# akashsengupta1997/STRAPS-3DHumanShapePose

Measured on AMD Instinct MI355X. Metric: bodies/sec, higher is better.
Workload: dtype fp32 (encoder convolutions as exact bf16x3 operand splits (six bf16 products per term); in-step SMPL blend contraction and skinning as 3-product fp16 splits (fp16x3_lbs: 22-bit operands); fp32 accumulate throughout)

## Files before the change

straps-3dhumanshapepose_amd/csrc/elementwise.hip:

```cpp
#include "common.h"

namespace {

__global__ __launch_bounds__(256) void pack_krsc_kernel(const float* __restrict__ src, float* __restrict__ dst, int O, int C, int R, int S) {
    const long long i = (long long)blockIdx.x * 256 + threadIdx.x;
    const long long n = (long long)O * C * R * S;
    if (i >= n) return;
    const int c = (int)(i % C);
    long long t = i / C;
    const int s = (int)(t % S); t /= S;
    const int r = (int)(t % R);
    const int o = (int)(t / R);
    dst[i] = src[(((long long)o * C + c) * R + r) * S + s];
}

__global__ __launch_bounds__(256) void pack_crsk_flip_kernel(const float* __restrict__ src, float* __restrict__ dst, int O, int C, int R, int S) {
    const long long i = (long long)blockIdx.x * 256 + threadIdx.x;
    const long long n = (long long)O * C * R * S;
    if (i >= n) return;
    const int o = (int)(i % O);
    long long t = i / O;
    const int s = (int)(t % S); t /= S;
    const int r = (int)(t % R);
    const int c = (int)(t / R);
// ... 102 lines not shown
            for (int idx = tid; idx < nc * nr * (PK_T / 4); idx += 256) {
                const int o = (idx & (PK_T / 4 - 1)) * 4;
                const int k = idx >> 3;
                const int c = nr == PK_RS ? k / PK_RS : k / nr, j = k - c * nr;
                if (o < no) {
                    const float* t = tile + o * PK_LD + c * PK_RS + j;
                    const f32x4 v = {t[0], t[PK_LD], t[2 * PK_LD], t[3 * PK_LD]};
                    store_planes4(c3, ps, D.first + wk_index(c0 + c, RS - 1 - (rs0 + j), o0 + o, D.c, D.o), v);
                }
            }
        }
        __syncthreads();
    }
}

__global__ void bn_fold_kernel(const float* __restrict__ g, const float* __restrict__ b, const float* __restrict__ mean,
                               const float* __restrict__ var, float eps, float* __restrict__ scale, float* __restrict__ shift, int C) {
    const int c = blockIdx.x * blockDim.x + threadIdx.x;
    if (c >= C) return;
    const float sc = g[c] / sqrtf(var[c] + eps);
    scale[c] = sc;
    shift[c] = fmaf(-mean[c], sc, b[c]);
}

__global__ __launch_bounds__(256) void maxpool_kernel(const float* __restrict__ x, float* __restrict__ y, int B, int H, int W, int C,
                                                      int Ho, int Wo) {
    const int C4 = C >> 2;
    const long long n = (long long)B * Ho * Wo * C4;
    for (long long i = (long long)blockIdx.x * 256 + threadIdx.x; i < n; i += (long long)gridDim.x * 256) {
        const int c4 = (int)(i % C4);
        long long t = i / C4;
        const int wo = (int)(t % Wo); t /= Wo;
        const int ho = (int)(t % Ho);
        const int b = (int)(t / Ho);
        f32x4 m = {-INFINITY, -INFINITY, -INFINITY, -INFINITY};
#pragma unroll
        for (int r = 0; r < 3; ++r) {
            const int hi = 2 * ho - 1 + r;
            if ((unsigned)hi >= (unsigned)H) continue;
#pragma unroll
            for (int s = 0; s < 3; ++s) {
                const int wi = 2 * wo - 1 + s;
                if ((unsigned)wi >= (unsigned)W) continue;
                const f32x4 v = *reinterpret_cast<const f32x4*>(x + (((long long)b * H + hi) * W + wi) * C + c4 * 4);
#pragma unroll
                for (int e = 0; e < 4; ++e)
                    if (v[e] > m[e] || v[e] != v[e]) m[e] = v[e];
            }
        }
        *reinterpret_cast<f32x4*>(y + i * 4) = m;
    }
}

__global__ __launch_bounds__(256) void gap_kernel(const float* __restrict__ x, float* __restrict__ y, int B, int HW, int C) {
    const long long i = (long long)blockIdx.x * 256 + threadIdx.x;
    if (i >= (long long)B * C) return;
    const int c = (int)(i % C);
    const long long b = i / C;
    const float* p = x + b * HW * C + c;
    float s = 0.f;
    for (int k = 0; k < HW; ++k) s += p[(long long)k * C];
    y[i] = s / (float)HW;
}

__global__ __launch_bounds__(256) void bn_stats_finalize_kernel(const float* __restrict__ part, int nblocks, int C, double count,
                                                               const float* __restrict__ gamma, const float* __restrict__ beta, float eps,
                                                               float momentum, float* __restrict__ rmean, float* __restrict__ rvar,
                                                               float* __restrict__ scale, float* __restrict__ shift,
                                                               float* __restrict__ smean, float* __restrict__ sinv) {
    int c;
    double s1, s2;
    if (bn_partials_sum4(part, nblocks, C, s1, s2, c)) {
        const double mean = s1 / count;
        double var = s2 / count - mean * mean;
        if (var < 0.0) var = 0.0;
        const float inv = (float)(1.0 / sqrt(var + (double)eps));
        const float sc = gamma[c] * inv;
        scale[c] = sc;
        shift[c] = fmaf(-(float)mean, sc, beta[c]);
        if (smean) smean[c] = (float)mean;
        if (sinv) sinv[c] = inv;
        if (rmean) {
            const double unbiased = count > 1.0 ? var * count / (count - 1.0) : var;
            rmean[c] = fmaf(momentum, (float)mean, (1.f - momentum) * rmean[c]);
            rvar[c] = fmaf(momentum, (float)unbiased, (1.f - momentum) * rvar[c]);
        }
    }
}

__global__ __launch_bounds__(256) void bn_apply_kernel(const float* __restrict__ x, const float* __restrict__ scale,
                                                       const float* __restrict__ shift, const float* __restrict__ res, int relu,
                                                       float* __restrict__ y, u16* __restrict__ planes, long long ps, long long n4, int C4,
                                                       unsigned* __restrict__ bits, int tiled) {
    const long long first = (long long)blockIdx.x * 256 + threadIdx.x, step = (long long)gridDim.x * 256;
    const long long rows = n4 / C4;
    auto body = [&](long long i, long long r, int c4, const f32x4& sc, const f32x4& sh) {
        f32x4 v = *reinterpret_cast<const f32x4*>(x + i * 4);
#pragma unroll
        for (int q = 0; q < 4; ++q) v[q] = fmaf(v[q], sc[q], sh[q]);
        if (res) v += *reinterpret_cast<const f32x4*>(res + i * 4);
        if (relu) { v[0] = fmaxf(v[0], 0.f); v[1] = fmaxf(v[1], 0.f); v[2] = fmaxf(v[2], 0.f); v[3] = fmaxf(v[3], 0.f); }
        if (y) *reinterpret_cast<f32x4*>(y + i * 4) = v;
        if (planes) store_planes4_cm(planes, ps, r, c4 * 4, rows, v);
        if (bits) {
            unsigned wd = ((v[0] > 0.f ? 1u : 0u) | (v[1] > 0.f ? 2u : 0u) | (v[2] > 0.f ? 4u : 0u) | (v[3] > 0.f ? 8u : 0u)) << ((c4 & 7) * 4);
            wd |= __shfl_xor(wd, 1, 64);
            wd |= __shfl_xor(wd, 2, 64);
            wd |= __shfl_xor(wd, 4, 64);
            if ((c4 & 7) == 0) bits[r * (C4 >> 3) + (c4 >> 3)] = wd;
        }
    };
    if (tiled) {
        const int l = threadIdx.x & 63, w = threadIdx.x >> 6, wcg = tiled, ncb = (C4 >> 4) / wcg, trows = 16 / wcg;
        const int c4 = ((int)(blockIdx.x % ncb) * wcg + w % wcg) * 16 + (l >> 5) * 8 + (l & 7);
// ... 54 lines not shown

extern "C" int straps_pack_conv_weights_batched(const straps_pack_desc_t* descs, int n, long long total, void* stream) {
    STRAPS_REQUIRE(descs && n > 0 && total > 0, "straps_pack_conv_weights_batched: bad arguments");
    long long blocks = (total + PK_T * PK_T * PK_RS - 1) / (PK_T * PK_T * PK_RS);
    if (blocks > 8192) blocks = 8192;
    hipLaunchKernelGGL(pack_batched_kernel, dim3((unsigned)blocks), dim3(256), 0, (hipStream_t)stream, descs, n, (u16*)nullptr, (u16*)nullptr, 0LL);
    STRAPS_CHECK_LAUNCH("pack_batched_kernel");
    return STRAPS_OK;
}

extern "C" int straps_pack_conv_weights_batched_x3(const straps_pack_desc_t* descs, int n, long long total, unsigned short* krsc_planes,
                                                   unsigned short* crsk_planes, long long plane_stride, void* stream) {
    STRAPS_REQUIRE(descs && n > 0 && total > 0, "straps_pack_conv_weights_batched_x3: bad arguments");
    STRAPS_REQUIRE(krsc_planes || crsk_planes, "straps_pack_conv_weights_batched_x3: no planes given (use straps_pack_conv_weights_batched)");
    STRAPS_REQUIRE(plane_stride >= total && plane_stride % 8 == 0, "straps_pack_conv_weights_batched_x3: plane_stride must be >= total and a multiple of 8");
    STRAPS_REQUIRE((reinterpret_cast<uintptr_t>(krsc_planes) & 15) == 0 && (reinterpret_cast<uintptr_t>(crsk_planes) & 15) == 0,
                   "straps_pack_conv_weights_batched_x3: plane buffers must be 16-byte aligned");
    long long blocks = (total + PK_T * PK_T * PK_RS - 1) / (PK_T * PK_T * PK_RS);
    if (blocks > 8192) blocks = 8192;
    hipLaunchKernelGGL(pack_batched_kernel, dim3((unsigned)blocks), dim3(256), 0, (hipStream_t)stream, descs, n, krsc_planes, crsk_planes, plane_stride);
    STRAPS_CHECK_LAUNCH("pack_batched_kernel");
    return STRAPS_OK;
}

extern "C" int straps_bn_fold(const float* gamma, const float* beta, const float* mean, const float* var, float eps, float* scale,
                              float* shift, int c, void* stream) {
    STRAPS_REQUIRE(gamma && beta && mean && var && scale && shift && c > 0, "straps_bn_fold: bad arguments");
    hipLaunchKernelGGL(bn_fold_kernel, dim3((c + 255) / 256), dim3(256), 0, (hipStream_t)stream, gamma, beta, mean, var, eps, scale, shift, c);
    STRAPS_CHECK_LAUNCH("bn_fold_kernel");
    return STRAPS_OK;
}

extern "C" int straps_bn_fold_stats(const float* gamma, const float* beta, const float* mean, const float* var, float eps, float* scale,
                                    float* shift, float* save_mean, float* save_invstd, int c, void* stream) {
    STRAPS_REQUIRE(gamma && beta && mean && var && scale && shift && save_mean && save_invstd && c > 0, "straps_bn_fold_stats: bad arguments");
    hipLaunchKernelGGL(bn_fold_stats_kernel, dim3((c + 255) / 256), dim3(256), 0, (hipStream_t)stream, gamma, beta, mean, var, eps, scale, shift, save_mean,
                       save_invstd, c);
    STRAPS_CHECK_LAUNCH("bn_fold_stats_kernel");
    return STRAPS_OK;
}

extern "C" int straps_maxpool_fwd(const float* x, float* y, int batch, int h, int w, int c, void* stream) {
    STRAPS_REQUIRE(x && y && batch > 0 && h > 0 && w > 0 && c > 0 && (c & 3) == 0, "straps_maxpool_fwd: bad arguments (c%%4 must be 0)");
    const int Ho = (h + 2 - 3) / 2 + 1, Wo = (w + 2 - 3) / 2 + 1;
    const long long n = (long long)batch * Ho * Wo * (c >> 2);
    hipLaunchKernelGGL(maxpool_kernel, dim3(capped_grid(n)), dim3(256), 0, (hipStream_t)stream, x, y, batch, h, w, c, Ho, Wo);
    STRAPS_CHECK_LAUNCH("maxpool_kernel");
    return STRAPS_OK;
}

extern "C" int straps_gap_fwd(const float* x, float* y, int batch, int hw, int c, void* stream) {
    STRAPS_REQUIRE(x && y && batch > 0 && hw > 0 && c > 0, "straps_gap_fwd: bad arguments");
    const long long n = (long long)batch * c;
    hipLaunchKernelGGL(gap_kernel, dim3((unsigned)((n + 255) / 256)), dim3(256), 0, (hipStream_t)stream, x, y, batch, hw, c);
    STRAPS_CHECK_LAUNCH("gap_kernel");
    return STRAPS_OK;
}

extern "C" int straps_bn_stats_finalize(const float* stats_partial, int nblocks, int c, long long count, const float* gamma,
                                        const float* beta, float eps, float momentum, float* running_mean, float* running_var,
                                        float* scale, float* shift, float* save_mean, float* save_invstd, void* stream) {
    STRAPS_REQUIRE(stats_partial && gamma && beta && scale && shift && nblocks > 0 && c > 0 && count > 0, "straps_bn_stats_finalize: bad arguments");
    STRAPS_REQUIRE((running_mean == nullptr) == (running_var == nullptr), "straps_bn_stats_finalize: running stats must be given together");
    hipLaunchKernelGGL(bn_stats_finalize_kernel, dim3((c + 3) / 4), dim3(256), 0, (hipStream_t)stream, stats_partial, nblocks, c, (double)count, gamma, beta,
                       eps, momentum, running_mean, running_var, scale, shift, save_mean, save_invstd);
    STRAPS_CHECK_LAUNCH("bn_stats_finalize_kernel");
    return STRAPS_OK;
}

extern "C" int straps_bn_apply(const float* x, const float* scale, const float* shift, const float* residual, int relu, float* y,
                               long long rows, int c, void* stream) {
    STRAPS_REQUIRE(x && scale && shift && y && rows > 0 && c > 0 && (c & 3) == 0, "straps_bn_apply: bad arguments (c%%4 must be 0)");
    const long long n4 = rows * (c >> 2);
    hipLaunchKernelGGL(bn_apply_kernel, dim3(capped_grid(n4)), dim3(256), 0, (hipStream_t)stream, x, scale, shift, residual, relu, y, (u16*)nullptr, 0LL, n4, c >> 2, (unsigned*)nullptr, 0);
    STRAPS_CHECK_LAUNCH("bn_apply_kernel");
    return STRAPS_OK;
}

static int bn_apply_x3_impl(const char* who, const float* x, const float* scale, const float* shift, const float* residual, int relu, float* y,
                            unsigned short* y_planes, long long plane_stride, unsigned* relu_bits, long long rows, int c, void* stream) {
    STRAPS_REQUIRE(x && scale && shift && (y_planes || y) && rows > 0 && c > 0 && (c & 31) == 0, "%s: bad arguments (c%%32 must be 0: chunk-major planes; c=%d)", who, c);
    STRAPS_REQUIRE(!y_planes || (plane_stride >= rows * c && plane_stride % 8 == 0), "%s: plane_stride must be >= rows*c and a multiple of 8", who);
    const long long n4 = rows * (c >> 2);
    const int tiled = straps_bn_tiled(rows, c >> 2);
    hipLaunchKernelGGL(bn_apply_kernel, dim3(tiled ? straps_bn_tiled_grid(rows, c >> 2, tiled) : straps_grid256_rows(n4, c >> 2)), dim3(256), 0, (hipStream_t)stream, x, scale, shift,
                       residual, relu, y, y_planes, plane_stride, n4, c >> 2, relu_bits, tiled);
    STRAPS_CHECK_LAUNCH("bn_apply_kernel");
    return STRAPS_OK;
}

extern "C" int straps_bn_apply_x3(const float* x, const float* scale, const float* shift, const float* residual, int relu, float* y,
                                  unsigned short* y_planes, long long plane_stride, long long rows, int c, void* stream) {
    return bn_apply_x3_impl("straps_bn_apply_x3", x, scale, shift, residual, relu, y, y_planes, plane_stride, nullptr, rows, c, stream);
}

extern "C" int straps_bn_apply_bits_x3(const float* x, const float* scale, const float* shift, const float* residual, float* y,
                                       unsigned short* y_planes, long long plane_stride, unsigned* relu_bits, long long rows, int c, void* stream) {
    STRAPS_REQUIRE(relu_bits, "straps_bn_apply_bits_x3: null bit buffer");
    return bn_apply_x3_impl("straps_bn_apply_bits_x3", x, scale, shift, residual, 1, y, y_planes, plane_stride, relu_bits, rows, c, stream);
}
```

straps-3dhumanshapepose_amd/csrc/ief.hip:

```cpp
#include "common.h"

namespace {

constexpr int LW = 8;
__global__ __launch_bounds__(64 * LW) void linear_kernel(const float* __restrict__ x, int ldx, const float* __restrict__ w, int ldw,
                                                     const float* __restrict__ bias, const float* addend, float* out, int ldo,
                                                     int M, int N, int K, int relu) {
    __shared__ float red[LW][32][33];
    const int tid = threadIdx.x, lane = tid & 63, wave = tid >> 6;
    const int m0 = blockIdx.y * 32, n0 = blockIdx.x * 32;
    const int i = lane & 31, h = lane >> 5;
    const int mr = min(m0 + i, M - 1);
    const float* xp = x + (long long)mr * ldx + 4 * h;
    const float* wp = w + (long long)(n0 + i) * ldw + 4 * h;
    f32x16 acc;
#pragma unroll
    for (int r = 0; r < 16; ++r) acc[r] = 0.f;
    const int G = K >> 3;
#pragma unroll 4
    for (int g = wave; g < G; g += LW) {
        const f32x4 a = *reinterpret_cast<const f32x4*>(xp + 8 * g);
        const f32x4 b = *reinterpret_cast<const f32x4*>(wp + 8 * g);
#pragma unroll
        for (int e = 0; e < 4; ++e) acc = mfma32(a[e], b[e], acc);
    }
#pragma unroll
    for (int r = 0; r < 16; ++r) red[wave][mfma_row(r, lane)][i] = acc[r];
    __syncthreads();
#pragma unroll
    for (int q = 0; q < 1024 / (64 * LW); ++q) {
        const int idx = tid + 64 * LW * q;
        const int row = idx >> 5, col = idx & 31;
        const int m = m0 + row, n = n0 + col;
        if (m < M && n < N) {
            float v = ((red[0][row][col] + red[1][row][col]) + (red[2][row][col] + red[3][row][col])) +
                      ((red[4][row][col] + red[5][row][col]) + (red[6][row][col] + red[7][row][col]));
            if (bias) v += bias[n];
            if (addend) v += addend[(long long)m * ldo + n];
            if (relu) v = fmaxf(v, 0.f);
            out[(long long)m * ldo + n] = v;
        }
    }
}

__global__ __launch_bounds__(256) void broadcast_rows_kernel(const float* __restrict__ row, int cols, float* __restrict__ dst,
                                                             int ld_dst, int m) {
    const long long i = (long long)blockIdx.x * 256 + threadIdx.x;
    if (i >= (long long)m * ld_dst) return;
    const int c = (int)(i % ld_dst);
    dst[i] = c < cols ? row[c] : 0.f;
}

struct GemmBatch {
    straps_gemm_desc_t d[STRAPS_GEMM_MULTI_MAX];
};

__global__ __launch_bounds__(64 * LW) void gemm_multi_kernel(GemmBatch batch) {
    const straps_gemm_desc_t& p = batch.d[blockIdx.z];
    const int M = p.m, N = p.n, K = p.k;
    const int m0 = blockIdx.y * 32, n0 = blockIdx.x * 32;
    if (m0 >= M || n0 >= N) return;
    __shared__ float red[LW][32][33];
    const int lane = threadIdx.x & 63, wave = threadIdx.x >> 6;
    const int i = lane & 31, h = lane >> 5;
    const int mr = min(m0 + i, M - 1), nr = min(n0 + i, N - 1);
    const float* ap = p.a + (long long)mr * p.sam;
    const float* bp = p.b + (long long)nr * p.sbn;
    const long long sak = p.sak, sbk = p.sbk;
    f32x16 acc;
#pragma unroll
    for (int q = 0; q < 16; ++q) acc[q] = 0.f;
    const int G = (K + 7) >> 3;
    for (int g = wave; g < G; g += 2 * LW) {
        float av[8], bv[8];
#pragma unroll
        for (int u = 0; u < 2; ++u) {
#pragma unroll
            for (int e = 0; e < 4; ++e) {
                const int k = (g + LW * u) * 8 + 4 * h + e;
                const bool ok = k < K;
                av[u * 4 + e] = ok ? ap[(long long)k * sak] : 0.f;
                bv[u * 4 + e] = ok ? bp[(long long)k * sbk] : 0.f;
            }
        }
#pragma unroll
        for (int e = 0; e < 8; ++e) acc = mfma32(av[e], bv[e], acc);
    }
#pragma unroll
    for (int q = 0; q < 16; ++q) red[wave][mfma_row(q, lane)][i] = acc[q];
    __syncthreads();
#pragma unroll
    for (int q = 0; q < 1024 / (64 * LW); ++q) {
        const int idx = threadIdx.x + 64 * LW * q;
        const int row = idx >> 5, col = idx & 31;
        const int m = m0 + row, n = n0 + col;
        if (m < M && n < N) {
            float v = ((red[0][row][col] + red[1][row][col]) + (red[2][row][col] + red[3][row][col])) +
                      ((red[4][row][col] + red[5][row][col]) + (red[6][row][col] + red[7][row][col]));
            if (p.addend) v += p.addend[(long long)m * p.ldadd + n];
            if (p.mask) v = p.mask[(long long)m * p.ldmask + n] > 0.f ? v : 0.f;
            float* o = p.c + (long long)m * p.ldc + n;
            *o = p.accumulate ? *o + v : v;
            if (p.c2) {
                float* o2 = p.c2 + (long long)m * p.ldc2 + n;
                *o2 = p.accumulate2 ? *o2 + v : v;
            }
        }
    }
}

__global__ __launch_bounds__(256) void ief_pack_kernel(const float* __restrict__ fc1, const float* __restrict__ fc3, float* __restrict__ w1f,
                                                       float* __restrict__ w1e, float* __restrict__ w3, int F, int P, int H1, int H2, int ld_e, int p_pad) {
    const long long n1 = (long long)H1 * F, n2 = (long long)H1 * ld_e, n3 = (long long)p_pad * H2;
    for (long long i = (long long)blockIdx.x * 256 + threadIdx.x; i < n1 + n2 + n3; i += (long long)gridDim.x * 256) {
        if (i < n1) {
            const int r = (int)(i / F), c = (int)(i - (long long)r * F);
            w1f[i] = fc1[(long long)r * (F + P) + c];
        } else if (i < n1 + n2) {
            const long long j = i - n1;
            const int r = (int)(j / ld_e), c = (int)(j - (long long)r * ld_e);
            w1e[j] = c < P ? fc1[(long long)r * (F + P) + F + c] : 0.f;
        } else {
            const long long j = i - n1 - n2;
            const int r = (int)(j / H2);
            w3[j] = r < P ? fc3[j] : 0.f;
        }
    }
}

}

extern "C" int straps_gemm_multi(const straps_gemm_desc_t* descs_host, int n, void* stream) {
    STRAPS_REQUIRE(descs_host && n >= 1 && n <= STRAPS_GEMM_MULTI_MAX, "straps_gemm_multi: need 1..%d problem descriptors (host memory)", STRAPS_GEMM_MULTI_MAX);
    GemmBatch batch;
    int gx = 0, gy = 0;
    for (int i = 0; i < n; ++i) {
        const straps_gemm_desc_t& d = descs_host[i];
        STRAPS_REQUIRE(d.a && d.b && d.c && d.m > 0 && d.n > 0 && d.k > 0, "straps_gemm_multi: problem %d: null operand or empty shape (m=%d n=%d k=%d)", i, d.m, d.n, d.k);
        batch.d[i] = d;
        gx = (d.n + 31) / 32 > gx ? (d.n + 31) / 32 : gx;
        gy = (d.m + 31) / 32 > gy ? (d.m + 31) / 32 : gy;
    }
    for (int i = n; i < STRAPS_GEMM_MULTI_MAX; ++i) batch.d[i] = descs_host[0];
    hipLaunchKernelGGL(gemm_multi_kernel, dim3(gx, gy, n), dim3(64 * LW), 0, (hipStream_t)stream, batch);
    STRAPS_CHECK_LAUNCH("gemm_multi_kernel");
    return STRAPS_OK;
}

extern "C" int straps_ief_pack(const float* fc1_w, const float* fc3_w, float* w1f, float* w1e, float* w3, int f, int p, int h1, int h2,
                               int ld_e, void* stream) {
    STRAPS_REQUIRE(fc1_w && fc3_w && w1f && w1e && w3, "straps_ief_pack: null pointer");
    STRAPS_REQUIRE(f > 0 && p > 0 && h1 > 0 && h2 > 0 && ld_e >= p, "straps_ief_pack: bad shape (f=%d p=%d h1=%d h2=%d ld_e=%d)", f, p, h1, h2, ld_e);
    const int p_pad = (p + 31) / 32 * 32;
    const long long total = (long long)h1 * f + (long long)h1 * ld_e + (long long)p_pad * h2;
    const int blocks = (int)((total + 255) / 256 < 2048 ? (total + 255) / 256 : 2048);
    hipLaunchKernelGGL(ief_pack_kernel, dim3(blocks), dim3(256), 0, (hipStream_t)stream, fc1_w, fc3_w, w1f, w1e, w3, f, p, h1, h2, ld_e, p_pad);
    STRAPS_CHECK_LAUNCH("ief_pack_kernel");
    return STRAPS_OK;
}

extern "C" int straps_linear_fwd(const float* x, int ldx, const float* w, int ldw, const float* bias, const float* addend,
                                 float* out, int ldo, int m, int n, int kdim, int relu, void* stream) {
    STRAPS_REQUIRE(x && w && out, "straps_linear_fwd: null pointer");
    STRAPS_REQUIRE(m > 0 && n > 0 && kdim > 0, "straps_linear_fwd: empty problem m=%d n=%d k=%d", m, n, kdim);
    STRAPS_REQUIRE((kdim & 7) == 0 && (ldx & 3) == 0 && (ldw & 3) == 0 && ldx >= kdim && ldw >= kdim,
                   "straps_linear_fwd: need kdim%%8==0, ldx%%4==0, ldw%%4==0 (kdim=%d ldx=%d ldw=%d)", kdim, ldx, ldw);
    STRAPS_REQUIRE(((uintptr_t)x & 15) == 0 && ((uintptr_t)w & 15) == 0, "straps_linear_fwd: x and w must be 16-byte aligned");
    dim3 grid((n + 31) / 32, (m + 31) / 32);
    hipLaunchKernelGGL(linear_kernel, grid, dim3(64 * LW), 0, (hipStream_t)stream, x, ldx, w, ldw, bias, addend, out, ldo, m, n, kdim, relu);
    STRAPS_CHECK_LAUNCH("linear_kernel");
    return STRAPS_OK;
}

extern "C" int straps_broadcast_rows(const float* row, int cols, float* dst, int ld_dst, int m, void* stream) {
    STRAPS_REQUIRE(row && dst && cols > 0 && ld_dst >= cols && m > 0, "straps_broadcast_rows: bad arguments");
    const long long n = (long long)m * ld_dst;
    hipLaunchKernelGGL(broadcast_rows_kernel, dim3((unsigned)((n + 255) / 256)), dim3(256), 0, (hipStream_t)stream, row, cols, dst, ld_dst, m);
    STRAPS_CHECK_LAUNCH("broadcast_rows_kernel");
    return STRAPS_OK;
}
```

straps-3dhumanshapepose_amd/csrc/raster.hip:

```cpp
#include "common.h"

#pragma clang fp contract(off)

namespace {

__global__ __launch_bounds__(256) STRAPS_NO_PACKED_FP32 void raster_project_kernel(const float* __restrict__ verts, const float* __restrict__ K,
                                                             const float* __restrict__ R, const float* __restrict__ t,
                                                             float* __restrict__ ndc, long long n, int nverts, int cam_per_body,
                                                             float orig, const float* __restrict__ noise_u, float noise_lo,
                                                             float noise_scale) {
    const long long i = (long long)blockIdx.x * 256 + threadIdx.x;
    if (i >= n) return;
    const long long b = i / nverts;
    const float* Kb = K + (cam_per_body ? b * 9 : 0);
    const float* Rb = R + (cam_per_body ? b * 9 : 0);
    const float* tb = t + b * 3;
    float x = verts[i * 3 + 0], y = verts[i * 3 + 1];
    const float z = verts[i * 3 + 2];
    if (noise_u) {
        x = x + (noise_scale * noise_u[i * 2 + 0] + noise_lo);
        y = y + (noise_scale * noise_u[i * 2 + 1] + noise_lo);
    }
    const float xc = ((Rb[0] * x + Rb[1] * y) + Rb[2] * z) + tb[0];
    const float yc = ((Rb[3] * x + Rb[4] * y) + Rb[5] * z) + tb[1];
    const float zc = ((Rb[6] * x + Rb[7] * y) + Rb[8] * z) + tb[2];
    const float den = zc + 1e-9f;
    const float xn = xc / den, yn = yc / den;
    const float u = (Kb[0] * xn + Kb[1] * yn) + Kb[2];
    float v = (Kb[3] * xn + Kb[4] * yn) + Kb[5];
    v = orig - v;
    const float half = orig / 2.f;
    ndc[i * 3 + 0] = 2.f * (u - half) / orig;
    ndc[i * 3 + 1] = 2.f * (v - half) / orig;
    ndc[i * 3 + 2] = zc;
}

__device__ __forceinline__ float edge_fn(float ax, float ay, float bx, float by, float px, float py) {
    return (px - ax) * (by - ay) - (py - ay) * (bx - ax);
}

#ifdef STRAPS_RASTER_CHECK_LOADS
__device__ unsigned g_raster_report[1 + 4 * 64];
#endif

template <int G>
__global__ __launch_bounds__(256) STRAPS_NO_PACKED_FP32 void raster_face_kernel(const float* __restrict__ ndc, const int32_t* __restrict__ faces,
                                                          unsigned long long* __restrict__ zbuf, long long n, int nverts,
                                                          int nfaces, int wh, float near, float far) {
    const bool pow2 = (wh & (wh - 1)) == 0;
    const float inv_wh = 1.f / (float)wh;
#if defined(STRAPS_RASTER_WRITE_TABLE) && !defined(STRAPS_RASTER_LDS_TABLE)
    extern __shared__ float sample[];
    for (int k = threadIdx.x; k < wh; k += 256) sample[k] = (float)(2 * k + 1 - wh) / (float)wh;
    __syncthreads();
#endif
#ifdef STRAPS_RASTER_DUMMY_BARRIER
    __syncthreads();
#endif
#ifdef STRAPS_RASTER_LDS_TABLE
    extern __shared__ float sample[];
    for (int k = threadIdx.x; k < wh; k += 256) sample[k] = (float)(2 * k + 1 - wh) / (float)wh;
    __syncthreads();
#endif
    const long long gid = (long long)blockIdx.x * 256 + threadIdx.x;
    const long long i = gid / G;
    const int sub = (int)(gid & (G - 1));
    if (i >= n) return;
    const long long b = i / nfaces;
    const int f = (int)(i - b * nfaces);
    const int i0 = faces[f * 3 + 0], i1 = faces[f * 3 + 1], i2 = faces[f * 3 + 2];
    if ((unsigned)i0 >= (unsigned)nverts || (unsigned)i1 >= (unsigned)nverts || (unsigned)i2 >= (unsigned)nverts) return;
    const float* p0 = ndc + (b * nverts + i0) * 3;
    const float* p1 = ndc + (b * nverts + i1) * 3;
    const float* p2 = ndc + (b * nverts + i2) * 3;
    const float x0 = p0[0], y0 = p0[1], z0 = p0[2];
    const float x1 = p1[0], y1 = p1[1], z1 = p1[2];
    const float x2 = p2[0], y2 = p2[1], z2 = p2[2];
    const float area = edge_fn(x0, y0, x1, y1, x2, y2);
    if (!(fabsf(area) > 1e-12f)) return;
    const float fw = (float)wh;
    const float xmin = fminf(x0, fminf(x1, x2)), xmax = fmaxf(x0, fmaxf(x1, x2));
    const float ymin = fminf(y0, fminf(y1, y2)), ymax = fmaxf(y0, fmaxf(y1, y2));
    if (!(xmax >= -1.f && xmin <= 1.f && ymax >= -1.f && ymin <= 1.f)) return;
    int xa = (int)floorf((fmaxf(xmin, -1.f) * fw + fw - 1.f) * 0.5f), xb = (int)ceilf((fminf(xmax, 1.f) * fw + fw - 1.f) * 0.5f);
    int ya = (int)floorf((fmaxf(ymin, -1.f) * fw + fw - 1.f) * 0.5f), yb = (int)ceilf((fminf(ymax, 1.f) * fw + fw - 1.f) * 0.5f);
    xa = xa < 0 ? 0 : xa; ya = ya < 0 ? 0 : ya;
    xb = xb > wh - 1 ? wh - 1 : xb; yb = yb > wh - 1 ? wh - 1 : yb;
    if (xb < xa || yb < ya) return;
    unsigned long long* zb = zbuf + b * (long long)wh * wh;
    const int bw = xb - xa + 1;
    int xi = xa + sub, yi = ya;
    while (xi > xb) { xi -= bw; ++yi; }
    for (; yi <= yb;) {
        {
            float yp, xp;
#ifdef STRAPS_RASTER_LDS_TABLE
            if (wh > 0) {
                yp = sample[yi];
                xp = sample[xi];
            } else
#endif
            if (pow2) {
                yp = (float)(2 * yi + 1 - wh) * inv_wh;
                xp = (float)(2 * xi + 1 - wh) * inv_wh;
            } else {
                yp = (float)(2 * yi + 1 - wh) / (float)wh;
                xp = (float)(2 * xi + 1 - wh) / (float)wh;
            }
            const float e0 = edge_fn(x1, y1, x2, y2, xp, yp);
            const float e1 = edge_fn(x2, y2, x0, y0, xp, yp);
            const float e2 = edge_fn(x0, y0, x1, y1, xp, yp);
            const bool in = (e0 >= 0.f && e1 >= 0.f && e2 >= 0.f) || (e0 <= 0.f && e1 <= 0.f && e2 <= 0.f);
            if (in) {
            float w0 = e0 / area, w1 = e1 / area, w2 = e2 / area;
            w0 = fminf(fmaxf(w0, 0.f), 1.f); w1 = fminf(fmaxf(w1, 0.f), 1.f); w2 = fminf(fmaxf(w2, 0.f), 1.f);
            const float ws = (w0 + w1) + w2;
            w0 = w0 / ws; w1 = w1 / ws; w2 = w2 / ws;
            const float zp = 1.f / ((w0 / z0 + w1 / z1) + w2 / z2);
            if (zp > near && zp < far) {
                const unsigned long long key = ((unsigned long long)__float_as_uint(zp) << 32) | (unsigned)f;
                atomicMin(zb + (long long)yi * wh + xi, key);
            }
            }
        }
        xi += G;
        while (xi > xb) { xi -= bw; ++yi; }
    }
#ifdef STRAPS_RASTER_CHECK_LOADS
    {
        const volatile float* q0 = p0; const volatile float* q1 = p1; const volatile float* q2 = p2;
        const float r[9] = {q0[0], q0[1], q0[2], q1[0], q1[1], q1[2], q2[0], q2[1], q2[2]};
        const float h[9] = {x0, y0, z0, x1, y1, z1, x2, y2, z2};
        for (int e = 0; e < 9; ++e)
            if (__float_as_uint(r[e]) != __float_as_uint(h[e])) {
                const unsigned k = atomicAdd(g_raster_report, 1u);
                if (k < 64) {
                    g_raster_report[1 + 4 * k + 0] = blockIdx.x; g_raster_report[1 + 4 * k + 1] = threadIdx.x | ((unsigned)e << 16) | ((unsigned)f << 20);
                    g_raster_report[1 + 4 * k + 2] = __float_as_uint(h[e]); g_raster_report[1 + 4 * k + 3] = __float_as_uint(r[e]);
                }
            }
    }
#endif
}

__global__ __launch_bounds__(256) void raster_resolve_kernel(const unsigned long long* __restrict__ zbuf,
                                                             const uint8_t* __restrict__ face_parts, float* __restrict__ parts,
                                                             float* __restrict__ depth, long long n, int wh, float far) {
    const long long i = (long long)blockIdx.x * 256 + threadIdx.x;
    if (i >= n) return;
    const long long b = i / ((long long)wh * wh);
    const int rem = (int)(i - b * (long long)wh * wh);
    const int row = rem / wh, col = rem - row * wh;
    const unsigned long long key = zbuf[b * (long long)wh * wh + (long long)(wh - 1 - row) * wh + col];
    const bool hit = key != ~0ULL;
    if (parts) parts[i] = hit ? (float)face_parts[(unsigned)(key & 0xffffffffULL)] : 0.f;
    if (depth) depth[i] = hit ? __uint_as_float((unsigned)(key >> 32)) : far;
}

}

int straps_fill_bytes(void* ptr, size_t bytes, unsigned char value, hipStream_t st);

extern "C" size_t straps_rasterize_workspace_bytes(long long batch, int nverts, int wh) {
    if (batch <= 0 || nverts <= 0 || wh <= 0) return 0;
    return (size_t)batch * ((size_t)wh * wh * sizeof(unsigned long long) + (size_t)nverts * 3 * sizeof(float));
}

extern "C" int straps_rasterize_parts(const float* verts, const int32_t* faces, const uint8_t* face_parts, const float* cam_K,
                                      const float* cam_R, const float* cam_t, float* parts, float* depth, void* workspace,
                                      long long batch, int nverts, int nfaces, int wh, int cam_per_body, float near, float far,
                                      const float* vert_noise_u, double noise_lo, double noise_hi, void* stream) {
    STRAPS_REQUIRE(verts && faces && face_parts && cam_K && cam_R && cam_t && workspace, "straps_rasterize_parts: null pointer");
    STRAPS_REQUIRE(parts || depth, "straps_rasterize_parts: neither parts nor depth requested");
    STRAPS_REQUIRE(batch > 0 && nverts > 0 && nfaces > 0 && wh > 0 && wh <= 4096, "straps_rasterize_parts: bad sizes (batch %lld, %d verts, %d faces, wh %d)",
                   batch, nverts, nfaces, wh);
    STRAPS_REQUIRE(far > near && near >= 0.f, "straps_rasterize_parts: need 0 <= near < far");
    hipStream_t st = (hipStream_t)stream;
    unsigned long long* zbuf = (unsigned long long*)workspace;
    float* ndc = (float*)(zbuf + batch * (long long)wh * wh);
    {
        const int rc = straps_fill_bytes(zbuf, (size_t)batch * wh * wh * sizeof(unsigned long long), 0xff, st);
        if (rc != STRAPS_OK) return rc;
    }
    const long long nv = batch * nverts, nf = batch * nfaces, np = batch * (long long)wh * wh;
    STRAPS_REQUIRE((nv + 255) / 256 < (1LL << 31) && (nf * 16 + 255) / 256 < (1LL << 31) && (np + 255) / 256 < (1LL << 31), "straps_rasterize_parts: batch too large for one launch");
    hipLaunchKernelGGL(raster_project_kernel, dim3((unsigned)((nv + 255) / 256)), dim3(256), 0, st, verts, cam_K, cam_R, cam_t, ndc, nv, nverts,
                       cam_per_body, (float)wh, vert_noise_u, (float)noise_lo, (float)(noise_hi - noise_lo));
    STRAPS_CHECK_LAUNCH("raster_project_kernel");
    static const int lanes = STRAPS_TOOL_ENV_INT("STRAPS_RASTER_LANES", 16);
#if defined(STRAPS_RASTER_LDS_TABLE) || defined(STRAPS_RASTER_WRITE_TABLE) || defined(STRAPS_RASTER_DUMMY_LDS)
    static const int lds_extra = STRAPS_TOOL_ENV_INT("STRAPS_RASTER_LDS_EXTRA", 0);
#define STRAPS_RASTER_LDS_BYTES ((size_t)wh * sizeof(float) + (size_t)lds_extra)
#else
#define STRAPS_RASTER_LDS_BYTES 0
#endif
#define STRAPS_RASTER_LAUNCH(G) hipLaunchKernelGGL(raster_face_kernel<G>, dim3((unsigned)((nf * G + 255) / 256)), dim3(256), STRAPS_RASTER_LDS_BYTES, st, ndc, faces, zbuf, nf, nverts, nfaces, wh, near, far)
    if (lanes == 1) STRAPS_RASTER_LAUNCH(1);
    else if (lanes == 2) STRAPS_RASTER_LAUNCH(2);
    else if (lanes == 4) STRAPS_RASTER_LAUNCH(4);
    else if (lanes == 8) STRAPS_RASTER_LAUNCH(8);
    else if (lanes == 32) STRAPS_RASTER_LAUNCH(32);
    else if (lanes == 64) STRAPS_RASTER_LAUNCH(64);
    else STRAPS_RASTER_LAUNCH(16);
#undef STRAPS_RASTER_LAUNCH
    STRAPS_CHECK_LAUNCH("raster_face_kernel");
    hipLaunchKernelGGL(raster_resolve_kernel, dim3((unsigned)((np + 255) / 256)), dim3(256), 0, st, zbuf, face_parts, parts, depth, np, wh, far);
    STRAPS_CHECK_LAUNCH("raster_resolve_kernel");
    return STRAPS_OK;
}

#ifdef STRAPS_TOOLS
namespace {
__global__ __launch_bounds__(256) void lds_occupier_kernel(int microseconds, unsigned* sink) {
    extern __shared__ unsigned occ[];
    if (threadIdx.x == 0) occ[0] = blockIdx.x;
    __syncthreads();
    const unsigned long long t0 = __builtin_amdgcn_s_memrealtime();
    while (__builtin_amdgcn_s_memrealtime() - t0 < (unsigned long long)microseconds * 100ull) __builtin_amdgcn_s_sleep(32);
    if (threadIdx.x == 0 && occ[0] == 0xffffffffu) sink[0] = 1;
}
}
namespace {
typedef __bf16 tool_bf16x8 __attribute__((ext_vector_type(8)));
template <int MFMA>
__device__ __forceinline__ void lds_frag_reader_body(unsigned* __restrict__ sink, int trips) {
    extern __shared__ __attribute__((aligned(16))) unsigned fr_lds[];
    const int tid = threadIdx.x, lane = tid & 63, wave = tid >> 6;
    for (int i = tid; i < 147 * 256; i += 256) fr_lds[i] = 0x3f803f80u ^ (unsigned)(i * 2654435761u >> 20);
    __syncthreads();
    const unsigned short* As = reinterpret_cast<const unsigned short*>(fr_lds);
    const int wm = wave >> 1, wn = wave & 1;
    int fo[2];
    for (int kk = 0; kk < 2; ++kk) fo[kk] = (lane & 31) * 32 + (((kk * 2 + (lane >> 5)) ^ (((lane & 31) >> 3) & 3)) << 3);
    f32x16 c[2][2];
    for (int i = 0; i < 2; ++i) for (int j = 0; j < 2; ++j) for (int r = 0; r < 16; ++r) c[i][j][r] = 0.f;
    unsigned acc = 0;
    int stage = 0;
    float keep[MFMA == 2 ? 230 : 1];
    for (int q = 0; q < (MFMA == 2 ? 230 : 1); ++q) keep[q] = (float)(lane + q);
    for (int t = 0; t < trips; ++t) {
        if (MFMA == 2) {
#pragma unroll
            for (int q = 0; q < (MFMA == 2 ? 230 : 1); ++q) asm volatile("" : "+v"(keep[q]));
        }
        const unsigned short* Ab = As + (stage * 3 * 256 + wm * 64) * 32;
        const unsigned short* Bb = As + (stage * 3 * 256 + 128 + wn * 64) * 32;
#pragma unroll
        for (int kk = 0; kk < 2; ++kk) {
            tool_bf16x8 a[2][3], b[2][3];
#pragma unroll
            for (int pl = 0; pl < 3; ++pl)
#pragma unroll
                for (int i = 0; i < 2; ++i) {
                    a[i][pl] = *reinterpret_cast<const tool_bf16x8*>(Ab + (pl * 256 + i * 32) * 32 + fo[kk]);
                    b[i][pl] = *reinterpret_cast<const tool_bf16x8*>(Bb + (pl * 256 + i * 32) * 32 + fo[kk]);
                }
            if (MFMA) {
                constexpr int TA[6] = {1, 0, 2, 0, 1, 0}, TB[6] = {1, 2, 0, 1, 0, 0};
#pragma unroll
// ... 60 lines not shown
```

Baseline: 8155.

## Vectorize and deepen K-loop loads in batched GEMM; unroll global average pool

Measured after the change: 8185, median of 6. Within noise of the previous version (+0.4%).

```diff
diff --git a/straps-3dhumanshapepose_amd/csrc/elementwise.hip b/straps-3dhumanshapepose_amd/csrc/elementwise.hip
--- a/straps-3dhumanshapepose_amd/csrc/elementwise.hip
+++ b/straps-3dhumanshapepose_amd/csrc/elementwise.hip
@@ -178,14 +178,28 @@
     }
 }
 
-__global__ __launch_bounds__(256) void gap_kernel(const float* __restrict__ x, float* __restrict__ y, int B, int HW, int C) {
-    const long long i = (long long)blockIdx.x * 256 + threadIdx.x;
+template <int T>
+__device__ __forceinline__ float gap_span(const float* __restrict__ p, long long C, float s) {
+    float v[T];
+#pragma unroll
+    for (int j = 0; j < T; ++j) v[j] = p[j * C];
+#pragma unroll
+    for (int j = 0; j < T; ++j) s += v[j];
+    return s;
+}
+
+constexpr int GAP_THREADS = 64;
+__global__ __launch_bounds__(GAP_THREADS) void gap_kernel(const float* __restrict__ x, float* __restrict__ y, int B, int HW, int C) {
+    const long long i = (long long)blockIdx.x * GAP_THREADS + threadIdx.x;
     if (i >= (long long)B * C) return;
     const int c = (int)(i % C);
     const long long b = i / C;
     const float* p = x + b * HW * C + c;
     float s = 0.f;
-    for (int k = 0; k < HW; ++k) s += p[(long long)k * C];
+    int k = 0;
+    for (; k + 64 <= HW; k += 64) s = gap_span<64>(p + (long long)k * C, C, s);
+    for (; k + 8 <= HW; k += 8) s = gap_span<8>(p + (long long)k * C, C, s);
+    for (; k < HW; ++k) s += p[(long long)k * C];
     y[i] = s / (float)HW;
 }
 
@@ -346,7 +360,7 @@
 extern "C" int straps_gap_fwd(const float* x, float* y, int batch, int hw, int c, void* stream) {
     STRAPS_REQUIRE(x && y && batch > 0 && hw > 0 && c > 0, "straps_gap_fwd: bad arguments");
     const long long n = (long long)batch * c;
-    hipLaunchKernelGGL(gap_kernel, dim3((unsigned)((n + 255) / 256)), dim3(256), 0, (hipStream_t)stream, x, y, batch, hw, c);
+    hipLaunchKernelGGL(gap_kernel, dim3((unsigned)((n + GAP_THREADS - 1) / GAP_THREADS)), dim3(GAP_THREADS), 0, (hipStream_t)stream, x, y, batch, hw, c);
     STRAPS_CHECK_LAUNCH("gap_kernel");
     return STRAPS_OK;
 }
diff --git a/straps-3dhumanshapepose_amd/csrc/ief.hip b/straps-3dhumanshapepose_amd/csrc/ief.hip
--- a/straps-3dhumanshapepose_amd/csrc/ief.hip
+++ b/straps-3dhumanshapepose_amd/csrc/ief.hip
@@ -55,6 +55,45 @@
     straps_gemm_desc_t d[STRAPS_GEMM_MULTI_MAX];
 };
 
+template <int T, bool AV, bool BV>
+__device__ __forceinline__ void k_groups(const float* __restrict__ ap, long long sak, const float* __restrict__ bp, long long sbk, int g, f32x16& acc) {
+    f32x4 a[T], b[T];
+#pragma unroll
+    for (int j = 0; j < T; ++j) {
+        const int k = 8 * (g + LW * j);
+        if (AV) {
+            a[j] = *reinterpret_cast<const f32x4*>(ap + k);
+        } else {
+#pragma unroll
+            for (int e = 0; e < 4; ++e) a[j][e] = ap[(long long)(k + e) * sak];
+        }
+        if (BV) {
+            b[j] = *reinterpret_cast<const f32x4*>(bp + k);
+        } else {
+#pragma unroll
+            for (int e = 0; e < 4; ++e) b[j][e] = bp[(long long)(k + e) * sbk];
+        }
+    }
+    __builtin_amdgcn_sched_barrier(0);
+#pragma unroll
+    for (int j = 0; j < T; ++j)
+#pragma unroll
+        for (int e = 0; e < 4; ++e) acc = mfma32(a[j][e], b[j][e], acc);
+}
+
+template <bool AV, bool BV, int TOP>
+__device__ __forceinline__ void k_groups_all(const float* __restrict__ ap, long long sak, const float* __restrict__ bp, long long sbk, int wave, int G,
+                                             f32x16& acc) {
+    int g = wave;
+    for (; g + (TOP - 1) * LW < G; g += TOP * LW) k_groups<TOP, AV, BV>(ap, sak, bp, sbk, g, acc);
+    if (TOP > 4)
+        for (; g + 3 * LW < G; g += 4 * LW) k_groups<4, AV, BV>(ap, sak, bp, sbk, g, acc);
+    if (TOP > 2)
+        for (; g + LW < G; g += 2 * LW) k_groups<2, AV, BV>(ap, sak, bp, sbk, g, acc);
+    for (; g < G; g += LW) k_groups<1, AV, BV>(ap, sak, bp, sbk, g, acc);
+}
+
+template <int TV, int TS>
 __global__ __launch_bounds__(64 * LW) void gemm_multi_kernel(GemmBatch batch) {
     const straps_gemm_desc_t& p = batch.d[blockIdx.z];
     const int M = p.m, N = p.n, K = p.k;
@@ -71,7 +110,21 @@
 #pragma unroll
     for (int q = 0; q < 16; ++q) acc[q] = 0.f;
     const int G = (K + 7) >> 3;
-    for (int g = wave; g < G; g += 2 * LW) {
+    const bool whole = (K & 7) == 0;
+    if (whole) {
+        const bool av = sak == 1 && ((uintptr_t)p.a & 15) == 0 && (p.sam & 3) == 0;
+        const bool bv = sbk == 1 && ((uintptr_t)p.b & 15) == 0 && (p.sbn & 3) == 0;
+        const float* a4 = ap + 4 * h * sak;
+        const float* b4 = bp + 4 * h * sbk;
+        if (av && bv) k_groups_all<true, true, TV>(a4, 1, b4, 1, wave, G, acc);
+        else if (av) k_groups_all<true, false, TS>(a4, 1, b4, sbk, wave, G, acc);
+        else k_groups_all<false, false, TS>(a4, sak, b4, sbk, wave, G, acc);
+        if (wave < G && (((G - 1 - wave) / LW) & 1) == 0) {
+#pragma unroll
+            for (int e = 0; e < 4; ++e) acc = mfma32(0.f, 0.f, acc);
+        }
+    }
+    for (int g = whole ? G : wave; g < G; g += 2 * LW) {
         float av[8], bv[8];
 #pragma unroll
         for (int u = 0; u < 2; ++u) {
@@ -134,15 +187,20 @@
     STRAPS_REQUIRE(descs_host && n >= 1 && n <= STRAPS_GEMM_MULTI_MAX, "straps_gemm_multi: need 1..%d problem descriptors (host memory)", STRAPS_GEMM_MULTI_MAX);
     GemmBatch batch;
     int gx = 0, gy = 0;
+    bool whole = false;
     for (int i = 0; i < n; ++i) {
         const straps_gemm_desc_t& d = descs_host[i];
         STRAPS_REQUIRE(d.a && d.b && d.c && d.m > 0 && d.n > 0 && d.k > 0, "straps_gemm_multi: problem %d: null operand or empty shape (m=%d n=%d k=%d)", i, d.m, d.n, d.k);
         batch.d[i] = d;
+        whole = whole || (d.k & 7) == 0;
         gx = (d.n + 31) / 32 > gx ? (d.n + 31) / 32 : gx;
         gy = (d.m + 31) / 32 > gy ? (d.m + 31) / 32 : gy;
     }
     for (int i = n; i < STRAPS_GEMM_MULTI_MAX; ++i) batch.d[i] = descs_host[0];
-    hipLaunchKernelGGL(gemm_multi_kernel, dim3(gx, gy, n), dim3(64 * LW), 0, (hipStream_t)stream, batch);
+    if (gx * gy * n <= 256 && whole)
+        hipLaunchKernelGGL((gemm_multi_kernel<16, 8>), dim3(gx, gy, n), dim3(64 * LW), 0, (hipStream_t)stream, batch);
+    else
+        hipLaunchKernelGGL((gemm_multi_kernel<4, 2>), dim3(gx, gy, n), dim3(64 * LW), 0, (hipStream_t)stream, batch);
     STRAPS_CHECK_LAUNCH("gemm_multi_kernel");
     return STRAPS_OK;
 }
```

## Compact live faces per wave and scan pixels with wave-shared face setup

Applied to the files above, without the earlier changes.

Measured after the change: 8200 before, 8177 after. Within noise of the previous version (-0.3%).

```diff
diff --git a/straps-3dhumanshapepose_amd/csrc/raster.hip b/straps-3dhumanshapepose_amd/csrc/raster.hip
--- a/straps-3dhumanshapepose_amd/csrc/raster.hip
+++ b/straps-3dhumanshapepose_amd/csrc/raster.hip
@@ -3,15 +3,22 @@
 #pragma clang fp contract(off)
 
 namespace {
+
+#define RASTER_BODIES_Y 32768
+#ifndef RASTER_LANES_DEFAULT
+#define RASTER_LANES_DEFAULT 32
+#endif
+__device__ __forceinline__ unsigned raster_body() { return blockIdx.z * (unsigned)RASTER_BODIES_Y + blockIdx.y; }
 
 __global__ __launch_bounds__(256) STRAPS_NO_PACKED_FP32 void raster_project_kernel(const float* __restrict__ verts, const float* __restrict__ K,
                                                              const float* __restrict__ R, const float* __restrict__ t,
-                                                             float* __restrict__ ndc, long long n, int nverts, int cam_per_body,
+                                                             float* __restrict__ ndc, unsigned batch, int nverts, int cam_per_body,
                                                              float orig, const float* __restrict__ noise_u, float noise_lo,
                                                              float noise_scale) {
-    const long long i = (long long)blockIdx.x * 256 + threadIdx.x;
-    if (i >= n) return;
-    const long long b = i / nverts;
+    const unsigned vi = blockIdx.x * 256u + threadIdx.x;
+    const long long b = raster_body();
+    if (b >= batch || vi >= (unsigned)nverts) return;
+    const long long i = b * nverts + vi;
     const float* Kb = K + (cam_per_body ? b * 9 : 0);
     const float* Rb = R + (cam_per_body ? b * 9 : 0);
     const float* tb = t + b * 3;
@@ -43,8 +50,123 @@
 __device__ unsigned g_raster_report[1 + 4 * 64];
 #endif
 
-template <int G>
+__device__ __forceinline__ float lane_f32(int lane4, float v) { return __builtin_bit_cast(float, __builtin_amdgcn_ds_bpermute(lane4, __builtin_bit_cast(int, v))); }
+
+template <int G, bool SCAN>
 __global__ __launch_bounds__(256) STRAPS_NO_PACKED_FP32 void raster_face_kernel(const float* __restrict__ ndc, const int32_t* __restrict__ faces,
+                                                          unsigned long long* __restrict__ zbuf, unsigned batch, int nverts,
+                                                          int nfaces, int wh, float near, float far) {
+    static_assert(G >= 1 && G <= 64 && (G & (G - 1)) == 0, "lanes per face: a power of two up to the wave");
+    constexpr int NG = 64 / G;
+    const bool pow2 = (wh & (wh - 1)) == 0;
+    const float inv_wh = 1.f / (float)wh;
+    const unsigned b = raster_body();
+    const int lane = threadIdx.x & 63;
+    const int f0 = (int)(blockIdx.x * 256u + (threadIdx.x & ~63u));
+    if (b >= batch || f0 >= nfaces) return;
+    const float* vb = ndc + (long long)b * nverts * 3;
+
+    const int f = f0 + lane;
+    float x0 = 0.f, y0 = 0.f, z0 = 0.f, x1 = 0.f, y1 = 0.f, z1 = 0.f, x2 = 0.f, y2 = 0.f, z2 = 0.f, area = 0.f;
+    int box_a = 0, box_b = 0;
+    unsigned box_m = 0;
+    bool live = false;
+    if (f < nfaces) {
+        const int i0 = faces[f * 3 + 0], i1 = faces[f * 3 + 1], i2 = faces[f * 3 + 2];
+        if (!((unsigned)i0 >= (unsigned)nverts || (unsigned)i1 >= (unsigned)nverts || (unsigned)i2 >= (unsigned)nverts)) {
+            const float* p0 = vb + (long long)i0 * 3;
+            const float* p1 = vb + (long long)i1 * 3;
+            const float* p2 = vb + (long long)i2 * 3;
+            x0 = p0[0], y0 = p0[1], z0 = p0[2];
+            x1 = p1[0], y1 = p1[1], z1 = p1[2];
+            x2 = p2[0], y2 = p2[1], z2 = p2[2];
+            area = edge_fn(x0, y0, x1, y1, x2, y2);
+            const float fw = (float)wh;
+            const float xmin = fminf(x0, fminf(x1, x2)), xmax = fmaxf(x0, fmaxf(x1, x2));
+            const float ymin = fminf(y0, fminf(y1, y2)), ymax = fmaxf(y0, fmaxf(y1, y2));
+            if (fabsf(area) > 1e-12f
+                && (xmax >= -1.f && xmin <= 1.f && ymax >= -1.f && ymin <= 1.f)) {
+                int xa = (int)floorf((fmaxf(xmin, -1.f) * fw + fw - 1.f) * 0.5f), xb = (int)ceilf((fminf(xmax, 1.f) * fw + fw - 1.f) * 0.5f);
+                int ya = (int)floorf((fmaxf(ymin, -1.f) * fw + fw - 1.f) * 0.5f), yb = (int)ceilf((fminf(ymax, 1.f) * fw + fw - 1.f) * 0.5f);
+                xa = xa < 0 ? 0 : xa; ya = ya < 0 ? 0 : ya;
+                xb = xb > wh - 1 ? wh - 1 : xb; yb = yb > wh - 1 ? wh - 1 : yb;
+                if (!(xb < xa || yb < ya)) {
+                    live = true;
+                    box_a = xa | (ya << 16);
+                    box_b = xb | (yb << 16);
+                    box_m = (1u << 24) / (unsigned)(xb - xa + 1) + 1u;
+                }
+            }
+        }
+    }
+
+    const unsigned long long mask = __builtin_amdgcn_ballot_w64(live);
+    if (mask == 0ull) return;
+    const int nlive = __builtin_popcountll(mask);
+    const int rank = (int)__builtin_amdgcn_mbcnt_hi((unsigned)(mask >> 32), __builtin_amdgcn_mbcnt_lo((unsigned)mask, 0u));
+    const int slot = live ? rank : nlive + (lane - rank);
+    const int owner = __builtin_amdgcn_ds_permute(slot << 2, lane);
+
+    const int grp = lane / G, sub = lane & (G - 1);
+    unsigned long long* zb = zbuf + (long long)b * wh * wh;
+    for (int j0 = 0; j0 < nlive; j0 += NG) {
+        const bool has = j0 + grp < nlive;
+        const int src = __builtin_amdgcn_ds_bpermute((has ? j0 + grp : 0) << 2, owner);
+        const int s4 = src << 2;
+        const float fx0 = lane_f32(s4, x0), fy0 = lane_f32(s4, y0), fz0 = lane_f32(s4, z0);
+        const float fx1 = lane_f32(s4, x1), fy1 = lane_f32(s4, y1), fz1 = lane_f32(s4, z1);
+        const float fx2 = lane_f32(s4, x2), fy2 = lane_f32(s4, y2), fz2 = lane_f32(s4, z2);
+        const float farea = lane_f32(s4, area);
+        const int ba = __builtin_amdgcn_ds_bpermute(s4, box_a), bb = __builtin_amdgcn_ds_bpermute(s4, box_b);
+        const unsigned bm = (unsigned)__builtin_amdgcn_ds_bpermute(s4, (int)box_m);
+        if (!has) continue;
+        const int xa = ba & 0xffff, ya = ba >> 16, xb = bb & 0xffff, yb = bb >> 16;
+        const unsigned fid = (unsigned)(f0 + src);
+        const int bw = xb - xa + 1;
+        const int qg = (int)(((unsigned)G * bm) >> 24), rg = G - qg * bw;
+        const int q0 = (int)(((unsigned)sub * bm) >> 24);
+        int xi = xa + (sub - q0 * bw), yi = ya + q0;
+#define RASTER_NEXT_SAMPLE() do { xi += rg; yi += qg; if (xi > xb) { xi -= bw; ++yi; } } while (0)
+        for (;;) {
+            float e0 = 0.f, e1 = 0.f, e2 = 0.f;
+            bool in = false;
+            while (yi <= yb) {
+                float yp, xp;
+                if (pow2) {
+                    yp = (float)(2 * yi + 1 - wh) * inv_wh;
+                    xp = (float)(2 * xi + 1 - wh) * inv_wh;
+                } else {
+                    yp = (float)(2 * yi + 1 - wh) / (float)wh;
+                    xp = (float)(2 * xi + 1 - wh) / (float)wh;
+                }
+                e0 = edge_fn(fx1, fy1, fx2, fy2, xp, yp);
+                e1 = edge_fn(fx2, fy2, fx0, fy0, xp, yp);
+                e2 = edge_fn(fx0, fy0, fx1, fy1, xp, yp);
+                in = (e0 >= 0.f && e1 >= 0.f && e2 >= 0.f) || (e0 <= 0.f && e1 <= 0.f && e2 <= 0.f);
+                if (!SCAN || in) break;
+                RASTER_NEXT_SAMPLE();
+            }
+            if (SCAN ? __builtin_amdgcn_ballot_w64(yi <= yb) == 0ull : !(yi <= yb)) break;
+            if (in) {
+                float w0 = e0 / farea, w1 = e1 / farea, w2 = e2 / farea;
+                w0 = fminf(fmaxf(w0, 0.f), 1.f); w1 = fminf(fmaxf(w1, 0.f), 1.f); w2 = fminf(fmaxf(w2, 0.f), 1.f);
+                const float ws = (w0 + w1) + w2;
+                w0 = w0 / ws; w1 = w1 / ws; w2 = w2 / ws;
+                const float zp = 1.f / ((w0 / fz0 + w1 / fz1) + w2 / fz2);
+                if (zp > near && zp < far) {
+                    const unsigned long long key = ((unsigned long long)__builtin_bit_cast(unsigned, zp) << 32) | fid;
+                    (void)__hip_atomic_fetch_min(zb + (long long)yi * wh + xi, key, __ATOMIC_RELAXED, __HIP_MEMORY_SCOPE_AGENT);
+                }
+            }
+            if (yi <= yb) RASTER_NEXT_SAMPLE();
+        }
+#undef RASTER_NEXT_SAMPLE
+    }
+}
+
+#ifdef STRAPS_TOOLS
+template <int G, bool NOWAIT>
+__global__ __launch_bounds__(256) STRAPS_NO_PACKED_FP32 void raster_face_parent_kernel(const float* __restrict__ ndc, const int32_t* __restrict__ faces,
                                                           unsigned long long* __restrict__ zbuf, long long n, int nverts,
                                                           int nfaces, int wh, float near, float far) {
     const bool pow2 = (wh & (wh - 1)) == 0;
@@ -119,7 +241,8 @@
             const float zp = 1.f / ((w0 / z0 + w1 / z1) + w2 / z2);
             if (zp > near && zp < far) {
                 const unsigned long long key = ((unsigned long long)__float_as_uint(zp) << 32) | (unsigned)f;
-                atomicMin(zb + (long long)yi * wh + xi, key);
+                if (NOWAIT) (void)__hip_atomic_fetch_min(zb + (long long)yi * wh + xi, key, __ATOMIC_RELAXED, __HIP_MEMORY_SCOPE_AGENT);
+                else atomicMin(zb + (long long)yi * wh + xi, key);
             }
             }
         }
@@ -142,16 +265,18 @@
     }
 #endif
 }
+#endif
 
 __global__ __launch_bounds__(256) void raster_resolve_kernel(const unsigned long long* __restrict__ zbuf,
                                                              const uint8_t* __restrict__ face_parts, float* __restrict__ parts,
-                                                             float* __restrict__ depth, long long n, int wh, float far) {
-    const long long i = (long long)blockIdx.x * 256 + threadIdx.x;
-    if (i >= n) return;
-    const long long b = i / ((long long)wh * wh);
-    const int rem = (int)(i - b * (long long)wh * wh);
-    const int row = rem / wh, col = rem - row * wh;
-    const unsigned long long key = zbuf[b * (long long)wh * wh + (long long)(wh - 1 - row) * wh + col];
+                                                             float* __restrict__ depth, unsigned batch, int wh, float far) {
+    const unsigned px = blockIdx.x * 256u + threadIdx.x;
+    const unsigned uwh = (unsigned)wh;
+    const long long b = raster_body();
+    if (b >= batch || px >= uwh * uwh) return;
+    const unsigned row = px / uwh, col = px - row * uwh;
+    const long long i = b * (long long)(uwh * uwh) + px;
+    const unsigned long long key = zbuf[b * (long long)(uwh * uwh) + (uwh - 1 - row) * uwh + col];
     const bool hit = key != ~0ULL;
     if (parts) parts[i] = hit ? (float)face_parts[(unsigned)(key & 0xffffffffULL)] : 0.f;
     if (depth) depth[i] = hit ? __uint_as_float((unsigned)(key >> 32)) : far;
@@ -182,29 +307,58 @@
         const int rc = straps_fill_bytes(zbuf, (size_t)batch * wh * wh * sizeof(unsigned long long), 0xff, st);
         if (rc != STRAPS_OK) return rc;
     }
-    const long long nv = batch * nverts, nf = batch * nfaces, np = batch * (long long)wh * wh;
-    STRAPS_REQUIRE((nv + 255) / 256 < (1LL << 31) && (nf * 16 + 255) / 256 < (1LL << 31) && (np + 255) / 256 < (1LL << 31), "straps_rasterize_parts: batch too large for one launch");
-    hipLaunchKernelGGL(raster_project_kernel, dim3((unsigned)((nv + 255) / 256)), dim3(256), 0, st, verts, cam_K, cam_R, cam_t, ndc, nv, nverts,
+    const long long gy = batch < RASTER_BODIES_Y ? batch : RASTER_BODIES_Y, gz = (batch + gy - 1) / gy;
+    const long long bv = ((long long)nverts + 255) / 256, bf = ((long long)nfaces + 255) / 256, bp = ((long long)wh * wh + 255) / 256;
+    STRAPS_REQUIRE(gz <= 65535 && bv * gy * gz < (1LL << 31) && bf * gy * gz < (1LL << 31) && bp * gy * gz < (1LL << 31), "straps_rasterize_parts: batch too large for one launch");
+    const unsigned ubatch = (unsigned)batch;
+    hipLaunchKernelGGL(raster_project_kernel, dim3((unsigned)bv, (unsigned)gy, (unsigned)gz), dim3(256), 0, st, verts, cam_K, cam_R, cam_t, ndc, ubatch, nverts,
                        cam_per_body, (float)wh, vert_noise_u, (float)noise_lo, (float)(noise_hi - noise_lo));
     STRAPS_CHECK_LAUNCH("raster_project_kernel");
-    static const int lanes = STRAPS_TOOL_ENV_INT("STRAPS_RASTER_LANES", 16);
+#define STRAPS_RASTER_FACE_LAUNCH(G, S) hipLaunchKernelGGL(HIP_KERNEL_NAME(raster_face_kernel<G, S>), dim3((unsigned)bf, (unsigned)gy, (unsigned)gz), dim3(256), 0, st, ndc, faces, zbuf, ubatch, nverts, nfaces, wh, near, far)
+#ifndef STRAPS_TOOLS
+    STRAPS_RASTER_FACE_LAUNCH(RASTER_LANES_DEFAULT, true);
+#else
+    const int lanes = STRAPS_TOOL_ENV_INT("STRAPS_RASTER_LANES", 0);
+#if defined(STRAPS_RASTER_LDS_TABLE) || defined(STRAPS_RASTER_WRITE_TABLE) || defined(STRAPS_RASTER_DUMMY_LDS) || defined(STRAPS_RASTER_DUMMY_BARRIER) || defined(STRAPS_RASTER_CHECK_LOADS)
+    const int parent_form = STRAPS_TOOL_ENV_INT("STRAPS_RASTER_PARENT", 1);
+#else
+    const int parent_form = STRAPS_TOOL_ENV_INT("STRAPS_RASTER_PARENT", 0);
+#endif
+    if (!parent_form) {
+        const int scan = STRAPS_TOOL_ENV_INT("STRAPS_RASTER_SCAN", 1);
+#define STRAPS_RASTER_FACE_FORMS(G) do { if (scan) STRAPS_RASTER_FACE_LAUNCH(G, true); else STRAPS_RASTER_FACE_LAUNCH(G, false); } while (0)
+        if (lanes == 2) STRAPS_RASTER_FACE_FORMS(2);
+        else if (lanes == 4) STRAPS_RASTER_FACE_FORMS(4);
+        else if (lanes == 8) STRAPS_RASTER_FACE_FORMS(8);
+        else if (lanes == 16) STRAPS_RASTER_FACE_FORMS(16);
+        else if (lanes == 32) STRAPS_RASTER_FACE_FORMS(32);
+        else if (lanes == 64) STRAPS_RASTER_FACE_FORMS(64);
+        else STRAPS_RASTER_FACE_FORMS(RASTER_LANES_DEFAULT);
+#undef STRAPS_RASTER_FACE_FORMS
+    } else {
+    const long long nf = batch * nfaces;
+    STRAPS_REQUIRE((nf * 64 + 255) / 256 < (1LL << 31), "straps_rasterize_parts: batch too large for one launch of the parent form");
 #if defined(STRAPS_RASTER_LDS_TABLE) || defined(STRAPS_RASTER_WRITE_TABLE) || defined(STRAPS_RASTER_DUMMY_LDS)
     static const int lds_extra = STRAPS_TOOL_ENV_INT("STRAPS_RASTER_LDS_EXTRA", 0);
 #define STRAPS_RASTER_LDS_BYTES ((size_t)wh * sizeof(float) + (size_t)lds_extra)
 #else
 #define STRAPS_RASTER_LDS_BYTES 0
 #endif
-#define STRAPS_RASTER_LAUNCH(G) hipLaunchKernelGGL(raster_face_kernel<G>, dim3((unsigned)((nf * G + 255) / 256)), dim3(256), STRAPS_RASTER_LDS_BYTES, st, ndc, faces, zbuf, nf, nverts, nfaces, wh, near, far)
+#define STRAPS_RASTER_LAUNCH(G) hipLaunchKernelGGL(HIP_KERNEL_NAME(raster_face_parent_kernel<G, false>), dim3((unsigned)((nf * G + 255) / 256)), dim3(256), STRAPS_RASTER_LDS_BYTES, st, ndc, faces, zbuf, nf, nverts, nfaces, wh, near, far)
     if (lanes == 1) STRAPS_RASTER_LAUNCH(1);
     else if (lanes == 2) STRAPS_RASTER_LAUNCH(2);
     else if (lanes == 4) STRAPS_RASTER_LAUNCH(4);
     else if (lanes == 8) STRAPS_RASTER_LAUNCH(8);
     else if (lanes == 32) STRAPS_RASTER_LAUNCH(32);
     else if (lanes == 64) STRAPS_RASTER_LAUNCH(64);
+    else if (parent_form == 2) hipLaunchKernelGGL(HIP_KERNEL_NAME(raster_face_parent_kernel<16, true>), dim3((unsigned)((nf * 16 + 255) / 256)), dim3(256), STRAPS_RASTER_LDS_BYTES, st, ndc, faces, zbuf, nf, nverts, nfaces, wh, near, far);
     else STRAPS_RASTER_LAUNCH(16);
 #undef STRAPS_RASTER_LAUNCH
+    }
+#endif
+#undef STRAPS_RASTER_FACE_LAUNCH
     STRAPS_CHECK_LAUNCH("raster_face_kernel");
-    hipLaunchKernelGGL(raster_resolve_kernel, dim3((unsigned)((np + 255) / 256)), dim3(256), 0, st, zbuf, face_parts, parts, depth, np, wh, far);
+    hipLaunchKernelGGL(raster_resolve_kernel, dim3((unsigned)bp, (unsigned)gy, (unsigned)gz), dim3(256), 0, st, zbuf, face_parts, parts, depth, ubatch, wh, far);
     STRAPS_CHECK_LAUNCH("raster_resolve_kernel");
     return STRAPS_OK;
 }
```
